# batra-mlp-lab/visdial

Measured on NVIDIA B200. Metric: QA-rounds/sec mn-att-ques-im-hist+disc train step, higher is better.
Workload: dtype f16 operands + f16 saved state for the option LSTM, tf32 operands elsewhere; fp32 accumulate, fp32 cell state / gradients / optimiser

## Files before the change

### visdial_b200/csrc/enc_lstm.cu

```cuda
#include <cuda.h>
#include <cuda_fp16.h>
#include "../../include/visdial_b200.h"
#include "kernels.cuh"
#include "tc_ptx.cuh"

namespace vd {
namespace tc {

constexpr int EP_THREADS = 192;
constexpr int EP_STAGES = 6;
constexpr int EP_STAGE_BYTES = 128 * 64 * 2;
constexpr int EP_W_BYTES_MAX = 131072;
constexpr int EP_SMEM = EP_W_BYTES_MAX + EP_STAGES * EP_STAGE_BYTES + 1024 + 256;
constexpr int EP_HS = 32;
static_assert(EP_SMEM <= 227 * 1024, "persistent encoder LSTM: shared memory budget");

__host__ __device__ constexpr uint32_t ep_idesc_f16(int M, int N) {
  return (1u << 4) | ((uint32_t)(N >> 3) << 17) | ((uint32_t)(M >> 4) << 24);
}
__device__ __forceinline__ void ep_umma_f16(uint32_t tmem_d, uint64_t adesc, uint64_t bdesc, uint32_t idesc, uint32_t accum) {
  asm volatile(
      "{\n .reg .pred p;\n setp.ne.b32 p, %4, 0;\n tcgen05.mma.cta_group::1.kind::f16 [%0], %1, %2, %3, p;\n}"
      ::"r"(tmem_d), "l"(adesc), "l"(bdesc), "r"(idesc), "r"(accum) : "memory");
}
// ... 34 lines not shown
__device__ __forceinline__ void st32h(__half* p, const float* v) {
  asm volatile("st.global.v8.b32 [%0], {%1,%2,%3,%4,%5,%6,%7,%8};"
               ::"l"(p), "r"(ep_pack2(v[0], v[1])), "r"(ep_pack2(v[2], v[3])), "r"(ep_pack2(v[4], v[5])), "r"(ep_pack2(v[6], v[7])),
                 "r"(ep_pack2(v[8], v[9])), "r"(ep_pack2(v[10], v[11])), "r"(ep_pack2(v[12], v[13])), "r"(ep_pack2(v[14], v[15])) : "memory");
  asm volatile("st.global.v8.b32 [%0], {%1,%2,%3,%4,%5,%6,%7,%8};"
               ::"l"(p + 16), "r"(ep_pack2(v[16], v[17])), "r"(ep_pack2(v[18], v[19])), "r"(ep_pack2(v[20], v[21])), "r"(ep_pack2(v[22], v[23])),
                 "r"(ep_pack2(v[24], v[25])), "r"(ep_pack2(v[26], v[27])), "r"(ep_pack2(v[28], v[29])), "r"(ep_pack2(v[30], v[31])) : "memory");
}
__device__ __forceinline__ void zero32(float* d) {
#pragma unroll
  for (int e = 0; e < 32; ++e) d[e] = 0.f;
}
__device__ __forceinline__ void tmem_ld32(uint32_t taddr, float* v) {
  tmem_ld8(taddr, v); tmem_ld8(taddr + 8, v + 8); tmem_ld8(taddr + 16, v + 16); tmem_ld8(taddr + 24, v + 24);
}
__device__ __forceinline__ void tmem_st8(uint32_t taddr, const float* v) {
  asm volatile("tcgen05.st.sync.aligned.32x32b.x8.b32 [%0], {%1,%2,%3,%4,%5,%6,%7,%8};"
               ::"r"(taddr), "r"(__float_as_uint(v[0])), "r"(__float_as_uint(v[1])), "r"(__float_as_uint(v[2])), "r"(__float_as_uint(v[3])),
                 "r"(__float_as_uint(v[4])), "r"(__float_as_uint(v[5])), "r"(__float_as_uint(v[6])), "r"(__float_as_uint(v[7])) : "memory");
}
__device__ __forceinline__ void tmem_st32(uint32_t taddr, const float* v) {
  tmem_st8(taddr, v); tmem_st8(taddr + 8, v + 8); tmem_st8(taddr + 16, v + 16); tmem_st8(taddr + 24, v + 24);
}
__device__ __forceinline__ void tmem_st_wait() { asm volatile("tcgen05.wait::st.sync.aligned;" ::: "memory"); }

constexpr int EP_TRACE_SLOTS = 10;
__device__ __forceinline__ void ep_stamp(unsigned long long* trace, int T, int t, int slot, bool wall = false) {
  if (trace) {
    unsigned long long v;
    if (wall) asm volatile("mov.u64 %0, %%globaltimer;" : "=l"(v));
    else v = (unsigned long long)clock64();
    trace[((size_t)blockIdx.x * T + t) * EP_TRACE_SLOTS + slot] = v;
  }
}

enum { EP_CELL1 = 0, EP_PROJ = 1, EP_CELL2 = 2 };

struct EncFwdParams {
  int T, R, H, RB;
// ... 645 lines not shown
```

### visdial_b200/csrc/engine.cu

```cuda
#include "engine.h"
#include <string.h>
#include <math.h>

namespace vd {

Cfg parse_cfg(const vd_params* p) {
  VD_REQUIRE(p && p->encoder && p->decoder, VD_E_BADARG, "params / encoder / decoder is null");
  Cfg c;
  c.encoder = p->encoder; c.decoder = p->decoder;
  struct { const char* name; int enc; } known[] = {
      {"lf-ques", ENC_LF_QUES}, {"lf-ques-im-hist", ENC_LF_QIH}, {"hrea-ques-im-hist", ENC_HREA}, {"mn-att-ques-im-hist", ENC_MN_ATT},
      {"lf-ques-im", ENC_LF_QI}, {"lf-ques-hist", ENC_LF_QH}, {"hre-ques-hist", ENC_HRE_QH}, {"hre-ques-im-hist", ENC_HRE_QIH},
      {"mn-ques-hist", ENC_MN_QH}, {"mn-ques-im-hist", ENC_MN_QIH}, {"lf-att-ques-im-hist", ENC_LF_ATT}};
  c.enc = -1;
  for (auto& k : known)
    if (c.encoder == k.name) c.enc = k.enc;
  VD_REQUIRE(c.enc >= 0, VD_E_BADARG, "unknown encoder (one of the eleven names of encoders/*.lua)");
  if (c.decoder == "disc") c.dec = DEC_DISC;
  else if (c.decoder == "gen") c.dec = DEC_GEN;
  else VD_REQUIRE(false, VD_E_BADARG, "unknown decoder (disc | gen)");
  c.V = p->vocabSize; c.E = p->embedSize; c.H = p->rnnHiddenSize; c.L = p->numLayers; c.F = p->imgFeatureSize;
  c.S = p->imgSpatialSize; c.IE = p->imgEmbedSize; c.Cm = p->commonEmbeddingSize; c.hops = p->numAttentionLayers;
  c.R = p->maxQuesCount; c.K = p->numOptions; c.dropout = p->dropout; c.gpuid = p->gpuid;
  c.useHist = c.encoder.find("hist") != std::string::npos;
// ... 123 lines not shown
  VD_CUDA_CHECK(cudaDeviceGetStreamPriorityRange(&prio_lo, &prio_hi));
  VD_CUDA_CHECK(cudaStreamCreateWithPriority(&cx.stream, cudaStreamNonBlocking, prio_hi));
  main_stream = cx.stream;
  VD_CUDA_CHECK(cudaStreamCreateWithPriority(&side_stream, cudaStreamNonBlocking, prio_hi));
  VD_CUDA_CHECK(cudaStreamCreateWithPriority(&main2_stream, cudaStreamNonBlocking, prio_hi));
  VD_CUDA_CHECK(cudaStreamCreateWithPriority(&side2_stream, cudaStreamNonBlocking, prio_hi));
  VD_CUDA_CHECK(cudaStreamCreateWithPriority(&main3_stream, cudaStreamNonBlocking, prio_hi));
  VD_CUDA_CHECK(cudaStreamCreateWithPriority(&side3_stream, cudaStreamNonBlocking, prio_hi));
  VD_CUDA_CHECK(cudaStreamCreateWithPriority(&opt_stream, cudaStreamNonBlocking, prio_lo));
  VD_CUDA_CHECK(cudaEventCreateWithFlags(&ev_fork, cudaEventDisableTiming));
  VD_CUDA_CHECK(cudaEventCreateWithFlags(&ev_join, cudaEventDisableTiming));
  VD_CUDA_CHECK(cudaEventCreateWithFlags(&ev_opt_fork, cudaEventDisableTiming));
  VD_CUDA_CHECK(cudaEventCreateWithFlags(&ev_opt_done, cudaEventDisableTiming));
  if (const char* s = getenv("VD_OPT_OVERLAP")) opt_overlap = atoi(s) != 0;
  if (const char* s = getenv("VD_OPT_RESERVE_SMS")) opt_reserve_sms = std::max(0, std::min(atoi(s), cx.sm_count - 16)) & ~1;
  size_t bytes = (size_t)nparams * sizeof(float);
  VD_CUDA_CHECK(cudaMalloc((void**)&W, bytes));
  VD_CUDA_CHECK(cudaMalloc((void**)&dW, bytes));
  VD_CUDA_CHECK(cudaMalloc((void**)&m, bytes));
  VD_CUDA_CHECK(cudaMalloc((void**)&v, bytes));
  VD_CUDA_CHECK(cudaMalloc((void**)&Wt, bytes));
  VD_CUDA_CHECK(cudaMemsetAsync(W, 0, bytes, cx.stream));
  VD_CUDA_CHECK(cudaMemsetAsync(dW, 0, bytes, cx.stream));
  VD_CUDA_CHECK(cudaMemsetAsync(m, 0, bytes, cx.stream));
  VD_CUDA_CHECK(cudaMemsetAsync(v, 0, bytes, cx.stream));
  VD_CUDA_CHECK(cudaMemsetAsync(Wt, 0, bytes, cx.stream));
  VD_CUDA_CHECK(cudaMalloc((void**)&scalars_dev, 64 * sizeof(float)));
  std::vector<int64_t> tab;
  for (auto& s : lay.segs) {
    if (s.init == VD_INIT_LSTM_W || s.init == VD_INIT_LINEAR_W) {
// ... 471 lines not shown
    else gemm_tn(V1, D, G, dP, G, nullptr, Ws, G, dWp(0), cfg.E, 1.f, nullptr, 0);
    VD_REQUIRE(dx_out == nullptr, VD_E_STATE, "projected-space embedding gradient: caller must not ask for dx");
    return;
  }
  if (pair16 && r.x16 && !r.gather && D % 64 == 0) {
    LaunchCtx::Scope sc(&cx, "gemm_wgrad", 2.0 * D * G * (double)TR, 2.0 * (double)TR * (D + G));
    gemm_atb16(cx, D, G, TR, r.x16, D, r.da16, G, dWs, G, nullptr);
  } else gemm_atb(D, G, TR, A, lda, r.gather, da, G, dWs, G);
  colsum_add(cx, dWp(r.wseg + 1), da, TR, G, G);
  if (dx_out) gemm_tn((int)TR, D, G, da, G, nullptr, Ws, G, dx_out, D, 0.f, nullptr, 0);
}

void Engine::lstm_backward(LstmRun& r, const float* dh_all, const float* dh_last, const float* dc_last, float* dx_out,
                           float* dh0_out, float* dc0_out) {
  lstm_backward_begin(r, dh_all, dh_last, dc_last);
  for (int t = r.T - 1; t >= 0; --t) lstm_backward_step(r, t);
  lstm_backward_end(r, dx_out, dh0_out, dc0_out);
}

void Engine::lstm_pair_backward(LstmRun& l1, LstmRun& l2, const float* dh_last2, const float* dc_last2, const float* dh_last1,
                                const float* dc_last1, float* dx1_out, cudaStream_t sa, cudaStream_t sb, cudaStream_t sc) {
  const int H = l2.H, G = 4 * l2.H;
  const int64_t R = l2.R;
  if (math_mode == VD_MATH_F16 && enc_persist_enabled() && l1.h16 && l2.h16 && l1.saved && l2.saved && l2.D == H && l1.T == l2.T &&
      enc_pair_shape_ok(R, H, cx.sm_count)) {
    const int T = l2.T;
    const int64_t TR = (int64_t)T * R;
    cx.stream = sa;
    l1.da = arena.get<float>(TR * G); l2.da = arena.get<float>(TR * G);
    l1.da16 = arena.get<__half>(TR * G); l2.da16 = arena.get<__half>(TR * G);
    __half* Whb2 = arena.get<__half>((int64_t)H * G);
// ... 746 lines not shown
```

### visdial_b200/csrc/engine.h

```cpp
#pragma once
#include <string>
#include <vector>
#include "../../include/visdial_b200.h"
#include "kernels.cuh"

namespace vd {

enum EncKind { ENC_LF_QUES = 0, ENC_LF_QIH = 1, ENC_HREA = 2, ENC_MN_ATT = 3, ENC_LF_QI = 4, ENC_LF_QH = 5, ENC_HRE_QH = 6, ENC_HRE_QIH = 7,
               ENC_MN_QH = 8, ENC_MN_QIH = 9, ENC_LF_ATT = 10 };
enum DecKind { DEC_DISC = 0, DEC_GEN = 1 };

struct Cfg {
  std::string encoder, decoder;
  int enc = 0, dec = 0;
  int V = 0, E = 300, H = 512, L = 2, F = 4096, S = 14, IE = 300, Cm = 512, hops = 1, R = 10, K = 100;
  float dropout = 0.5f;
  int gpuid = 0;
  bool useIm = false, useHist = false, att = false;
  bool fam_lf = false, fam_hre = false, fam_mn = false;
  bool hre_att = false;
  bool san = false;
  bool img_in_q = false;
  bool img_drop = false;
  bool mn_qi = false;
// ... 139 lines not shown
  void lstm_forward(LstmRun& r, bool save);
  void lstm_forward_begin(LstmRun& r, bool save);
  void lstm_forward_step(LstmRun& r, int t);
  void lstm_backward_begin(LstmRun& r, const float* dh_all, const float* dh_last, const float* dc_last);
  void lstm_backward_step(LstmRun& r, int t);
  void lstm_backward_end(LstmRun& r, float* dx_out, float* dh0_out, float* dc0_out);
  void lstm_pair_forward(LstmRun& l1, LstmRun& l2, cudaStream_t sa, cudaStream_t sb, cudaStream_t sc);
  void lstm_pair_backward(LstmRun& l1, LstmRun& l2, const float* dh_last2, const float* dc_last2, const float* dh_last1,
                          const float* dc_last1, float* dx1_out, cudaStream_t sa, cudaStream_t sb, cudaStream_t sc);
  void lstm_forward_xproj(LstmRun& r, int t);
  cudaStream_t main2_stream = nullptr, side2_stream = nullptr, main3_stream = nullptr, side3_stream = nullptr;
  cudaStream_t opt_stream = nullptr;
  cudaEvent_t ev_opt_fork = nullptr, ev_opt_done = nullptr;
  bool opt_overlap = true, opt_fwd_pending = false, opt_bwd_pending = false;
  int opt_reserve_sms = 16;
  float* opt_demb = nullptr;
  void options_forward_async();
  void join_options_backward();
  std::vector<cudaEvent_t> ev_pool;
  cudaEvent_t pool_event(size_t i);
  void lstm_backward(LstmRun& r, const float* dh_all, const float* dh_last, const float* dc_last, float* dx_out,
                     float* dh0_out, float* dc0_out);

  void encoder_forward(const vd_batch* b);
  void encoder_backward(const float* dEnc);
  float *qi_join = nullptr, *qi_proj = nullptr;
  const float* mn_query_in = nullptr;
  void mn_block_fwd(const float* qin, const float* h3, float* out);
  void mn_block_bwd(const float* dout, const float* out, float* dqin, float* dh3);
  void san_block_fwd(const float* u0);
// ... 30 lines not shown
```

### visdial_b200/csrc/kernels.cuh

```cuda
#pragma once
#include <algorithm>
#include <cuda_fp16.h>
#include "common.cuh"

namespace vd {

void gemm_tn_simt(LaunchCtx& cx, int M, int N, int K, const float* A, int64_t lda, const int32_t* a_gather,
                  const float* B, int64_t ldb, float* C, int64_t ldc, float beta, const float* bias, int act);
void gemm_atb_simt(LaunchCtx& cx, int M, int N, int64_t K, const float* A, int64_t lda, const int32_t* a_gather,
                   const float* B, int64_t ldb, float* C, int64_t ldc);
bool gemm_tn_tc(LaunchCtx& cx, int M, int N, int K, const float* A, int64_t lda, const int32_t* a_gather,
                const float* B, int64_t ldb, float* C, int64_t ldc, float beta, const float* bias, int act);
bool gemm_atb_tc(LaunchCtx& cx, int M, int N, int64_t K, const float* A, int64_t lda, const int32_t* a_gather,
                 const float* B, int64_t ldb, float* C, int64_t ldc);

int vocab_lse_nparts(int N);
bool vocab_lse_tc(LaunchCtx& cx, int M, int N, int K, const float* A, int64_t lda, const float* B, int64_t ldb, const float* bias,
                  const int32_t* tgt, float* part_max, float* part_sum, float* tgt_logit);
bool vocab_dlogits_tc(LaunchCtx& cx, int M, int N, int K, const float* A, int64_t lda, const float* B, int64_t ldb, const float* bias,
                      const int32_t* tgt, const int32_t* row_ids, const float* lse, float* C, int64_t ldc);
void vocab_lse_finish(LaunchCtx& cx, const float* part_max, const float* part_sum, int nparts, const float* tgt_logit,
                      const int32_t* tgt, const int32_t* row_ids, float* lse, float* out, float sign, int accumulate, int64_t rows);

void transpose_ids(LaunchCtx& cx, const int32_t* src, int32_t* dst, int64_t rows, int T);
// ... 79 lines not shown
bool lstm_step_fwd_tc(LaunchCtx& cx, int64_t R, int H, const float* h_prev, const float* WtS_h, int64_t ldw, const float* bias,
                      float* gates, int has_xproj, const float* ptable, const int32_t* tok, const float* c_prev, float* c_out,
                      float* h_out, const int32_t* mask_ids);
bool lstm_step_bwd_tc(LaunchCtx& cx, int64_t R, int H, const float* da_next, const float* Wh, const float* gsave,
                      const float* c_prev, const float* c_cur, const float* dh_ext, float* dc_carry, const int32_t* mask_ids,
                      float* da);
}

namespace vd {
bool lstm16_shape_ok(int64_t R, int H);
void lstm16_step_fwd(LaunchCtx& cx, int64_t R, int H, const __half* h_prev16, const __half* Wh16, const __half* ptable16,
                     const int32_t* tok, const float* bias, const float* c_prev, const int32_t* mask_ids, __half* gates16,
                     float* c_out, __half* h16_out, float* h32_out);
void lstm16_step_bwd(LaunchCtx& cx, int64_t R, int H, const __half* da_next16, const __half* Whb16, const __half* gates16,
                     const float* c_prev, const float* c_cur, float* dc_carry, const int32_t* mask_ids, __half* da16);
void lstm16_first_step(LaunchCtx& cx, int64_t R, int H, const __half* ptable16, const int32_t* tok, const float* bias,
                       const float* c_prev, const int32_t* mask_ids, __half* gates16, float* c_out, __half* h16_out, float* h32_out);
void lstm16_bwd_last(LaunchCtx& cx, int64_t R, int H, const __half* gates16, const float* c_prev, const float* c_cur,
                     const float* dh_last, const float* scale, const int32_t* mask_ids, float* dc_carry, __half* da16);
void cvt_f32_to_f16(LaunchCtx& cx, __half* dst, int64_t ldd, const float* src, int64_t lds, int64_t rows, int cols);
void pick_grad_scale(LaunchCtx& cx, const float* x, int64_t n, uint32_t* bits, float* scale2);
void segsum_rows16(LaunchCtx& cx, const __half* X, int64_t ldx, const int32_t* perm, const int32_t* sorted_tok, int64_t n,
                   float* out, int ncols, const float* inv_scale);
void gemm_atb16(LaunchCtx& cx, int M, int N, int64_t K, const __half* A, int64_t lda, const __half* B, int64_t ldb, float* C,
                int64_t ldc, const float* inv_scale);
bool enc_pair_shape_ok(int64_t R, int H, int sm_count);
void enc_pair_forward(LaunchCtx& cx, int T, int64_t R, int H, const __half* W1h16, const __half* W2cat16, const float* bias2,
                      const int32_t* mask, float* gates1, float* c1, float* h1, __half* h1_16, float* gates2, float* c2, float* h2,
                      __half* h2_16, int* flags);
void enc_pair_backward(LaunchCtx& cx, int T, int64_t R, int H, const __half* B1cat16, const __half* Whb2_16, const int32_t* mask,
// ... 7 lines not shown
```

### visdial_b200/csrc/lstm16.cu

```cuda
#include <cuda.h>
#include <cuda_fp16.h>
#include "../../include/visdial_b200.h"
#include "kernels.cuh"
#include "tc_ptx.cuh"

namespace vd {
namespace tc {

constexpr int BM16 = 128;
constexpr int BK16 = 64;
constexpr int UK16 = 16;
template <int MODE> struct EW16T { static constexpr int N = MODE == 0 ? 16 : 8; };
constexpr int STAGE16 = 32768;

__host__ __device__ constexpr uint32_t make_idesc_f16(int M, int N, int a_mn_major, int b_mn_major) {
  return (1u << 4) | ((uint32_t)a_mn_major << 15) | ((uint32_t)b_mn_major << 16) | ((uint32_t)(N >> 3) << 17) |
         ((uint32_t)(M >> 4) << 24);
}
__device__ __forceinline__ void umma_f16(uint32_t tmem_d, uint64_t adesc, uint64_t bdesc, uint32_t idesc, uint32_t accum) {
  asm volatile(
      "{\n .reg .pred p;\n setp.ne.b32 p, %4, 0;\n tcgen05.mma.cta_group::1.kind::f16 [%0], %1, %2, %3, p;\n}"
      ::"r"(tmem_d), "l"(adesc), "l"(bdesc), "r"(idesc), "r"(accum) : "memory");
}
__device__ __forceinline__ void umma_f16_cg2(uint32_t tmem_d, uint64_t adesc, uint64_t bdesc, uint32_t idesc, uint32_t accum) {
// ... 343 lines not shown
      tc_fence_before();
      __syncwarp();
      if (lane == 0) {
        if (!leader) mbar_arrive_cluster(mapa_u32(smem_u32(&tempty[buf]), 0));
        else mbar_arrive(&tempty[buf]);
      }
    }
    }
    if (lane == 0) asm volatile("cp.async.bulk.wait_group 0;" ::: "memory");
  }
  tc_fence_before();
  cluster_sync_all();
  if (warp == 1) { tc_fence_after(); tmem_dealloc_cg2(tmem_base, 2 * BN); }
}

constexpr int A16_KB = 64;
constexpr int A16_BN = 256;
constexpr int A16_THREADS = 192;
constexpr int A16_A_BYTES = 2 * A16_KB * 128;
constexpr int A16_B_BYTES = (A16_BN / 64) * A16_KB * 128;
constexpr int A16_STAGE = A16_A_BYTES + A16_B_BYTES;
constexpr int A16_STAGES = 4;
constexpr int A16_TOTAL = A16_STAGES * A16_STAGE + 1024 + 256;
struct Atb16Params { int M, N; int64_t K, k_per_split; float* C; int64_t ldc; const float* inv_scale; };

__global__ void __launch_bounds__(A16_THREADS, 1)
k_atb16(const __grid_constant__ CUtensorMap tmA, const __grid_constant__ CUtensorMap tmB, const Atb16Params p) {
  extern __shared__ uint8_t smem_raw[];
  uint8_t* smem = (uint8_t*)(((uintptr_t)smem_raw + 1023) & ~(uintptr_t)1023);
  uint64_t* full = (uint64_t*)(smem + A16_STAGES * A16_STAGE);
// ... 255 lines not shown
    snprintf(buf, sizeof(buf), "cuTensorMapEncodeTiled (lstm16) failed (%d): base %p rows %lld cols %lld ld %lld box %dx%d", (int)r, base,
             (long long)rows, (long long)cols, (long long)ld, box_rows, box_cols);
    throw CudaError(-3, buf);
  }
  return tm;
}
static CUtensorMap tmap_h(const __half* base, int64_t rows, int64_t cols, int64_t ld, int box_rows, int box_cols,
                          CUtensorMapSwizzle swz) {
  return make_tmap16(base, CU_TENSOR_MAP_DATA_TYPE_FLOAT16, 2, rows, cols, ld, box_rows, box_cols, swz);
}
static CUtensorMap tmap_f(const float* base, int64_t rows, int64_t cols, int64_t ld, int box_rows, int box_cols,
                          CUtensorMapSwizzle swz) {
  return make_tmap16(base, CU_TENSOR_MAP_DATA_TYPE_FLOAT32, 4, rows, cols, ld, box_rows, box_cols, swz);
}

template <int MODE>
static void launch16(LaunchCtx& cx, const CUtensorMap& tA, const CUtensorMap& tB, const Lstm16Maps& em, const Lstm16Params& p,
                     int num_tiles) {
  using C = Cfg16<MODE>;
  static bool attr_set = false;
  if (!attr_set) {
    VD_CUDA_CHECK(cudaFuncSetAttribute(k_lstm16<MODE>, cudaFuncAttributeMaxDynamicSharedMemorySize, C::TOTAL));
    attr_set = true;
  }
  const int pmax = cx.sms() / 2;
  int pairs = num_tiles;
  if (num_tiles > pmax) { const int rounds = cdiv(num_tiles, pmax); pairs = cdiv(num_tiles, rounds); }
  cudaLaunchConfig_t cfg = {};
  cfg.gridDim = dim3(2 * pairs);
  cfg.blockDim = dim3(C::THREADS);
  cfg.dynamicSmemBytes = C::TOTAL;
  cfg.stream = cx.stream;
  cudaLaunchAttribute at[1];
  at[0].id = cudaLaunchAttributeClusterDimension;
  at[0].val.clusterDim.x = 2; at[0].val.clusterDim.y = 1; at[0].val.clusterDim.z = 1;
  cfg.attrs = at; cfg.numAttrs = 1;
  VD_CUDA_CHECK(cudaLaunchKernelEx(&cfg, k_lstm16<MODE>, tA, tB, em, p));
  check_launch(cx, "k_lstm16");
}
// ... 23 lines not shown
void lstm16_step_bwd(LaunchCtx& cx, int64_t R, int H, const __half* da_next16, const __half* Whb16, const __half* gates16,
                     const float* c_prev, const float* c_cur, float* dc_carry, const int32_t* mask_ids, __half* da16) {
  using namespace tc;
  VD_REQUIRE(lstm16_shape_ok(R, H), VD_E_STATE, "lstm16_step_bwd: shape");
  Lstm16Params p = {};
  p.R = (int)R; p.H = H; p.gsave = gates16; p.c_prev = c_prev; p.c_cur = c_cur; p.dc_carry = dc_carry; p.mask_ids = mask_ids;
  CUtensorMap tA = tmap_h(da_next16, R, 4 * (int64_t)H, 4 * (int64_t)H, BM16, BK16, CU_TENSOR_MAP_SWIZZLE_128B);
  CUtensorMap tB = tmap_h(Whb16, H, 4 * (int64_t)H, 4 * (int64_t)H, 128, BK16, CU_TENSOR_MAP_SWIZZLE_128B);
  Lstm16Maps em;
  em.g16 = tmap_h(da16, R, 4 * (int64_t)H, 4 * (int64_t)H, 32, 16, CU_TENSOR_MAP_SWIZZLE_32B);
  em.c = tmap_f(dc_carry, R, H, H, 32, 16, CU_TENSOR_MAP_SWIZZLE_64B);
  em.h16 = em.c;
  launch16<1>(cx, tA, tB, em, p, cdiv(R, 2 * BM16) * (H / 256));
}

void lstm16_first_step(LaunchCtx& cx, int64_t R, int H, const __half* ptable16, const int32_t* tok, const float* bias,
                       const float* c_prev, const int32_t* mask_ids, __half* gates16, float* c_out, __half* h16_out, float* h32_out) {
  const int64_t n = R * (H / 8);
  tc::k_lstm16_first<<<(unsigned)((n + 255) / 256), 256, 0, cx.stream>>>(ptable16, tok, bias, c_prev, mask_ids, gates16, c_out,
                                                                          h16_out, h32_out, R, H);
  check_launch(cx, "k_lstm16_first");
}

void lstm16_bwd_last(LaunchCtx& cx, int64_t R, int H, const __half* gates16, const float* c_prev, const float* c_cur,
                     const float* dh_last, const float* scale, const int32_t* mask_ids, float* dc_carry, __half* da16) {
  const int64_t n = R * (H / 8);
  tc::k_lstm16_bwd_last<<<(unsigned)((n + 255) / 256), 256, 0, cx.stream>>>(gates16, c_prev, c_cur, dh_last, scale, mask_ids,
                                                                             dc_carry, da16, R, H);
  check_launch(cx, "k_lstm16_bwd_last");
}
// ... 25 lines not shown
  check_launch(cx, "k_segsum16");
}

void gemm_atb16(LaunchCtx& cx, int M, int N, int64_t K, const __half* A, int64_t lda, const __half* B, int64_t ldb, float* C,
                int64_t ldc, const float* inv_scale) {
  using namespace tc;
  VD_REQUIRE(M % 64 == 0 && N % 64 == 0 && K >= A16_KB && lda % 8 == 0 && ldb % 8 == 0, VD_E_STATE, "gemm_atb16: shape");
  const int tiles = cdiv(M, BM16) * cdiv(N, A16_BN);
  const int64_t cta_cap = cx.sm_budget > 0 ? cx.sm_budget : 2LL * cx.sm_count;
  int64_t splits = std::max<int64_t>(1, std::min<int64_t>(cta_cap / tiles, K / (A16_KB * 4)));
  int64_t kps = ((K + splits - 1) / splits + A16_KB - 1) / A16_KB * A16_KB;
  splits = (K + kps - 1) / kps;
  Atb16Params p = {M, N, K, kps, C, ldc, inv_scale};
  CUtensorMap tA = tmap_h(A, K, M, lda, A16_KB, 64, CU_TENSOR_MAP_SWIZZLE_128B),
              tB = tmap_h(B, K, N, ldb, A16_KB, 64, CU_TENSOR_MAP_SWIZZLE_128B);
  static bool attr_set = false;
  if (!attr_set) {
    VD_CUDA_CHECK(cudaFuncSetAttribute(k_atb16, cudaFuncAttributeMaxDynamicSharedMemorySize, A16_TOTAL));
    attr_set = true;
  }
  dim3 grid(tiles, (unsigned)splits);
  k_atb16<<<grid, A16_THREADS, A16_TOTAL, cx.stream>>>(tA, tB, p);
  check_launch(cx, "k_atb16");
}

}
```

### visdial_b200/csrc/tc_ptx.cuh

```cuda
#pragma once
#include <cuda.h>
#include <stdint.h>

namespace vd {
namespace tc {

__device__ __forceinline__ uint32_t smem_u32(const void* p) { return (uint32_t)__cvta_generic_to_shared(p); }

__device__ __forceinline__ void mbar_init(uint64_t* bar, uint32_t count) {
  asm volatile("mbarrier.init.shared::cta.b64 [%0], %1;" ::"r"(smem_u32(bar)), "r"(count));
}
__device__ __forceinline__ void mbar_expect_tx(uint64_t* bar, uint32_t bytes) {
  asm volatile("mbarrier.arrive.expect_tx.shared::cta.b64 _, [%0], %1;" ::"r"(smem_u32(bar)), "r"(bytes) : "memory");
}
__device__ __forceinline__ void mbar_arrive(uint64_t* bar) {
  asm volatile("mbarrier.arrive.shared::cta.b64 _, [%0];" ::"r"(smem_u32(bar)) : "memory");
}
__device__ __forceinline__ void mbar_wait(uint64_t* bar, uint32_t parity) {
  uint32_t done = 0, spins = 0;
  uint32_t addr = smem_u32(bar);
  while (!done) {
    asm volatile(
        "{\n .reg .pred p;\n mbarrier.try_wait.parity.shared::cta.b64 p, [%1], %2;\n selp.u32 %0, 1, 0, p;\n}"
        : "=r"(done) : "r"(addr), "r"(parity) : "memory");
// ... 51 lines not shown
  asm volatile("tcgen05.alloc.cta_group::2.sync.aligned.shared::cta.b32 [%0], %1;" ::"r"(smem_u32(dst_smem)), "r"(ncols) : "memory");
  asm volatile("tcgen05.relinquish_alloc_permit.cta_group::2.sync.aligned;" ::: "memory");
}
__device__ __forceinline__ void tmem_dealloc_cg2(uint32_t addr, uint32_t ncols) {
  asm volatile("tcgen05.dealloc.cta_group::2.sync.aligned.b32 %0, %1;" ::"r"(addr), "r"(ncols) : "memory");
}
__device__ __forceinline__ void umma_tf32_cg2(uint32_t tmem_d, uint64_t adesc, uint64_t bdesc, uint32_t idesc, uint32_t accum) {
  asm volatile(
      "{\n .reg .pred p;\n setp.ne.b32 p, %4, 0;\n tcgen05.mma.cta_group::2.kind::tf32 [%0], %1, %2, %3, p;\n}"
      ::"r"(tmem_d), "l"(adesc), "l"(bdesc), "r"(idesc), "r"(accum) : "memory");
}
__device__ __forceinline__ void umma_commit_cg2(uint64_t* bar) {
  asm volatile("tcgen05.commit.cta_group::2.mbarrier::arrive::one.shared::cluster.multicast::cluster.b64 [%0], %1;"
               ::"r"(smem_u32(bar)), "h"((uint16_t)3) : "memory");
}

__device__ __forceinline__ uint64_t make_desc(uint32_t saddr, uint32_t lbo_bytes, uint32_t sbo_bytes, uint32_t layout_type = 2) {
  uint64_t d = 0;
  d |= (uint64_t)((saddr & 0x3FFFF) >> 4);
  d |= (uint64_t)((lbo_bytes >> 4) & 0x3FFF) << 16;
  d |= (uint64_t)((sbo_bytes >> 4) & 0x3FFF) << 32;
  d |= (uint64_t)1 << 46;
  d |= (uint64_t)layout_type << 61;
  return d;
}
__host__ __device__ constexpr uint32_t make_idesc(int M, int N, int a_mn_major, int b_mn_major) {
  return (1u << 4) | (2u << 7) | (2u << 10) | ((uint32_t)a_mn_major << 15) | ((uint32_t)b_mn_major << 16) |
         ((uint32_t)(N >> 3) << 17) | ((uint32_t)(M >> 4) << 24);
}

__device__ __forceinline__ float fsigmoid(float x) { return __fdividef(1.f, 1.f + __expf(-x)); }
__device__ __forceinline__ float ftanh(float x) {
  float e = __expf(-2.f * fabsf(x));
  return copysignf(__fdividef(1.f - e, 1.f + e), x);
}

__device__ __forceinline__ const float* shfl_ptr(const float* p, int src_lane) {
  unsigned long long v = (unsigned long long)p;
  unsigned lo = __shfl_sync(0xffffffffu, (unsigned)v, src_lane), hi = __shfl_sync(0xffffffffu, (unsigned)(v >> 32), src_lane);
  return (const float*)(((unsigned long long)hi << 32) | lo);
}
__device__ __forceinline__ void tma_store_2d(const CUtensorMap* tm, const void* smem_src, int c0, int c1) {
  asm volatile("cp.async.bulk.tensor.2d.global.shared::cta.bulk_group [%0, {%2, %3}], [%1];"
               ::"l"(tm), "r"(smem_u32(smem_src)), "r"(c0), "r"(c1) : "memory");
}
__device__ __forceinline__ void fence_proxy_async_smem() { asm volatile("fence.proxy.async.shared::cta;" ::: "memory"); }
__device__ __forceinline__ void bulk_commit() { asm volatile("cp.async.bulk.commit_group;" ::: "memory"); }
__device__ __forceinline__ void bulk_wait_read0() { asm volatile("cp.async.bulk.wait_group.read 0;" ::: "memory"); }
__device__ __forceinline__ void red_add_v4(float* addr, float a, float b, float c, float d) {
  asm volatile("red.global.add.v4.f32 [%0], {%1, %2, %3, %4};" ::"l"(addr), "f"(a), "f"(b), "f"(c), "f"(d) : "memory");
}


typedef CUresult (*PFN_encodeTiled)(CUtensorMap*, CUtensorMapDataType, cuuint32_t, void*, const cuuint64_t*, const cuuint64_t*,
                                    const cuuint32_t*, const cuuint32_t*, CUtensorMapInterleave, CUtensorMapSwizzle,
                                    CUtensorMapL2promotion, CUtensorMapFloatOOBfill);
PFN_encodeTiled get_encode();
}
}
```

Baseline: 33870.

## Fuse f16 option-LSTM backward-through-time into one persistent cluster kernel

Replaces the per-timestep loop of f16 LSTM backward launches with a single persistent cluster kernel. Each step's recurrent GEMM (da_{t+1} x W_hh) runs on tcgen05 into tensor memory, and the pointwise gate gradients are computed in place, with the cell-gradient carry kept in tensor memory. Cross-CTA ordering between steps uses cluster mbarriers and TMA stores/loads. This removes T per-step launches and their global round trips for the carry, but needs the whole grid in one cluster set, adds complex cluster synchronisation, and has an environment fallback to the old path.

```diff
diff --git a/visdial_b200/csrc/enc_lstm.cu b/visdial_b200/csrc/enc_lstm.cu
--- a/visdial_b200/csrc/enc_lstm.cu
+++ b/visdial_b200/csrc/enc_lstm.cu
@@ -72,15 +72,9 @@
 __device__ __forceinline__ void tmem_ld32(uint32_t taddr, float* v) {
   tmem_ld8(taddr, v); tmem_ld8(taddr + 8, v + 8); tmem_ld8(taddr + 16, v + 16); tmem_ld8(taddr + 24, v + 24);
 }
-__device__ __forceinline__ void tmem_st8(uint32_t taddr, const float* v) {
-  asm volatile("tcgen05.st.sync.aligned.32x32b.x8.b32 [%0], {%1,%2,%3,%4,%5,%6,%7,%8};"
-               ::"r"(taddr), "r"(__float_as_uint(v[0])), "r"(__float_as_uint(v[1])), "r"(__float_as_uint(v[2])), "r"(__float_as_uint(v[3])),
-                 "r"(__float_as_uint(v[4])), "r"(__float_as_uint(v[5])), "r"(__float_as_uint(v[6])), "r"(__float_as_uint(v[7])) : "memory");
-}
 __device__ __forceinline__ void tmem_st32(uint32_t taddr, const float* v) {
   tmem_st8(taddr, v); tmem_st8(taddr + 8, v + 8); tmem_st8(taddr + 16, v + 16); tmem_st8(taddr + 24, v + 24);
 }
-__device__ __forceinline__ void tmem_st_wait() { asm volatile("tcgen05.wait::st.sync.aligned;" ::: "memory"); }
 
 constexpr int EP_TRACE_SLOTS = 10;
 __device__ __forceinline__ void ep_stamp(unsigned long long* trace, int T, int t, int slot, bool wall = false) {
diff --git a/visdial_b200/csrc/engine.cu b/visdial_b200/csrc/engine.cu
--- a/visdial_b200/csrc/engine.cu
+++ b/visdial_b200/csrc/engine.cu
@@ -161,6 +161,7 @@
   VD_CUDA_CHECK(cudaEventCreateWithFlags(&ev_opt_done, cudaEventDisableTiming));
   if (const char* s = getenv("VD_OPT_OVERLAP")) opt_overlap = atoi(s) != 0;
   if (const char* s = getenv("VD_OPT_RESERVE_SMS")) opt_reserve_sms = std::max(0, std::min(atoi(s), cx.sm_count - 16)) & ~1;
+  if (const char* s = getenv("VD_OPT_BPTT")) opt_bptt_fused = strcmp(s, "perstep") != 0;
   size_t bytes = (size_t)nparams * sizeof(float);
   VD_CUDA_CHECK(cudaMalloc((void**)&W, bytes));
   VD_CUDA_CHECK(cudaMalloc((void**)&dW, bytes));
@@ -662,7 +663,14 @@
 void Engine::lstm_backward(LstmRun& r, const float* dh_all, const float* dh_last, const float* dc_last, float* dx_out,
                            float* dh0_out, float* dc0_out) {
   lstm_backward_begin(r, dh_all, dh_last, dc_last);
-  for (int t = r.T - 1; t >= 0; --t) lstm_backward_step(r, t);
+  if (r.f16 && opt_bptt_fused && lstm16_bptt_ok(r.R, r.H, r.T)) {
+    const int H = r.H, T = r.T;
+    const double R = (double)r.R, G = 4.0 * H;
+    LaunchCtx::Scope sc(&cx, "lstm_step_bwd", (T - 1) * 2.0 * R * G * H, R * ((T - 1) * (2.0 * G + 8.0 * H + 2.0 * G) + 2.0 * G + 12.0 * H + 2.0 * G));
+    lstm16_bptt(cx, T, r.R, H, r.Whb16, r.gates16, r.c, r.c0, r.bw_dh_last, r.scale2, r.mask, r.da16);
+  } else {
+    for (int t = r.T - 1; t >= 0; --t) lstm_backward_step(r, t);
+  }
   lstm_backward_end(r, dx_out, dh0_out, dc0_out);
 }
 
diff --git a/visdial_b200/csrc/engine.h b/visdial_b200/csrc/engine.h
--- a/visdial_b200/csrc/engine.h
+++ b/visdial_b200/csrc/engine.h
@@ -177,6 +177,7 @@
   cudaEvent_t ev_opt_fork = nullptr, ev_opt_done = nullptr;
   bool opt_overlap = true, opt_fwd_pending = false, opt_bwd_pending = false;
   int opt_reserve_sms = 16;
+  bool opt_bptt_fused = true;
   float* opt_demb = nullptr;
   void options_forward_async();
   void join_options_backward();
diff --git a/visdial_b200/csrc/kernels.cuh b/visdial_b200/csrc/kernels.cuh
--- a/visdial_b200/csrc/kernels.cuh
+++ b/visdial_b200/csrc/kernels.cuh
@@ -117,6 +117,9 @@
                      float* c_out, __half* h16_out, float* h32_out);
 void lstm16_step_bwd(LaunchCtx& cx, int64_t R, int H, const __half* da_next16, const __half* Whb16, const __half* gates16,
                      const float* c_prev, const float* c_cur, float* dc_carry, const int32_t* mask_ids, __half* da16);
+bool lstm16_bptt_ok(int64_t R, int H, int T);
+void lstm16_bptt(LaunchCtx& cx,int T, int64_t R, int H, const __half* Whb16, const __half* gates16, const float* c, const float* c0,
+                 const float* dh_last, const float* scale, const int32_t* mask_ids, __half* da16);
 void lstm16_first_step(LaunchCtx& cx, int64_t R, int H, const __half* ptable16, const int32_t* tok, const float* bias,
                        const float* c_prev, const int32_t* mask_ids, __half* gates16, float* c_out, __half* h16_out, float* h32_out);
 void lstm16_bwd_last(LaunchCtx& cx, int64_t R, int H, const __half* gates16, const float* c_prev, const float* c_cur,
diff --git a/visdial_b200/csrc/lstm16.cu b/visdial_b200/csrc/lstm16.cu
--- a/visdial_b200/csrc/lstm16.cu
+++ b/visdial_b200/csrc/lstm16.cu
@@ -381,6 +381,213 @@
   if (warp == 1) { tc_fence_after(); tmem_dealloc_cg2(tmem_base, 2 * BN); }
 }
 
+struct BpttParams {
+  int R, H, T;
+  const __half* gates;
+  const float* c;
+  const float* c0;
+  const float* dh_last;
+  const float* scale;
+  const int32_t* mask;
+};
+
+__global__ void __launch_bounds__(Cfg16<1>::THREADS, 1)
+k_lstm16_bptt(const __grid_constant__ CUtensorMap tmA, const __grid_constant__ CUtensorMap tmB,
+              const __grid_constant__ CUtensorMap tmD, const BpttParams p) {
+  using C = Cfg16<1>;
+  constexpr int STAGES = C::STAGES;
+  constexpr int BN = 256;
+  const uint32_t rank = cluster_ctarank(), cs = cluster_nctarank();
+  const uint32_t lead = rank & ~1u;
+  const bool leader = rank == lead;
+  const uint16_t pair_mask = (uint16_t)(3u << lead);
+  const int sub = (int)(rank & 1), pair = (int)(rank >> 1);
+  extern __shared__ uint8_t smem_raw[];
+  uint8_t* smem = (uint8_t*)(((uintptr_t)smem_raw + 1023) & ~(uintptr_t)1023);
+  uint8_t* stg_all = smem + STAGES * STAGE16;
+  uint64_t* full = (uint64_t*)(stg_all + C::STG_BYTES);
+  uint64_t* empty = full + STAGES;
+  uint64_t* tfull = empty + STAGES;
+  uint64_t* tempty = tfull + 1;
+  uint64_t* ready = tempty + 1;
+  uint32_t* tmem_slot = (uint32_t*)(ready + 1);
+
+  const int warp = threadIdx.x >> 5, lane = threadIdx.x & 31;
+  const int H = p.H, T = p.T;
+  const int64_t R = p.R;
+  const int m0 = (int)(blockIdx.x / cs) * 2 * BM16 + sub * BM16;
+  const int n0 = pair * BN;
+  const int num_kb = 4 * H / BK16;
+
+  if (threadIdx.x == 0) {
+    for (int s = 0; s < STAGES; ++s) { mbar_init(&full[s], 1); mbar_init(&empty[s], 1); }
+    mbar_init(tfull, 1);
+    mbar_init(tempty, C::EW * 2);
+    mbar_init(ready, C::EW * cs);
+    asm volatile("fence.mbarrier_init.release.cluster;" ::: "memory");
+  }
+  cluster_sync_all();
+  if (warp == 1) tmem_alloc_cg2(tmem_slot, 2 * BN);
+  tc_fence_before();
+  __syncthreads();
+  tc_fence_after();
+  const uint32_t tmem_base = *tmem_slot;
+
+  if (warp == 0) {
+    if (lane == 0) {
+      int s = 0; uint32_t ph = 0;
+      for (int t = T - 2; t >= 0; --t) {
+        mbar_wait_acquire_cluster(ready, (uint32_t)(T - 2 - t) & 1);
+        fence_proxy_async_global();
+        for (int kb = 0; kb < num_kb; ++kb) {
+          mbar_wait(&empty[s], ph ^ 1);
+          uint8_t* sa = smem + s * STAGE16;
+          const uint32_t bar = mapa_u32(smem_u32(&full[s]), lead);
+          if (leader) mbar_expect_tx(&full[s], 2 * STAGE16);
+          tma_load_3d_cg2(sa, &tmA, bar, kb * BK16, m0, t + 1);
+          tma_load_2d_cg2(sa + 16384, &tmB, bar, kb * BK16, n0 + sub * 128);
+          if (++s == STAGES) { s = 0; ph ^= 1; }
+        }
+      }
+    }
+  } else if (warp == 1 && !leader) {
+  } else if (warp == 1) {
+    constexpr uint32_t idesc = make_idesc_f16(2 * BM16, BN, 0, 0);
+    int s = 0; uint32_t ph = 0;
+    for (int i = 0; i < T - 1; ++i) {
+      mbar_wait(tempty, ((uint32_t)i & 1) ^ 1);
+      tc_fence_after();
+      for (int kb = 0; kb < num_kb; ++kb) {
+        mbar_wait(&full[s], ph);
+        tc_fence_after();
+        if (lane == 0) {
+          const uint32_t sa = smem_u32(smem + s * STAGE16);
+          const uint64_t adesc = make_desc(sa, 16, 1024);
+          const uint64_t bdesc = make_desc(sa + 16384, 16, 1024);
+#pragma unroll
+          for (int k = 0; k < BK16 / UK16; ++k)
+            umma_f16_cg2(tmem_base, adesc + (uint64_t)(k * 2), bdesc + (uint64_t)(k * 2), idesc, (kb | k) ? 1u : 0u);
+          umma_commit_cg2_mask(&empty[s], pair_mask);
+          if (kb == num_kb - 1) umma_commit_cg2_mask(tfull, pair_mask);
+        }
+        __syncwarp();
+        if (++s == STAGES) { s = 0; ph ^= 1; }
+      }
+    }
+  } else {
+    constexpr int NSL = C::EW / 4, GPW = 256 / NSL / 16;
+    const int q = warp & 3;
+    const int half = (warp - 2) >> 2;
+    static_assert(C::EW * C::STG_PER_WARP <= STAGES * STAGE16, "second staging set must fit the pipeline stages");
+    uint8_t* const stg_a = stg_all + (warp - 2) * C::STG_PER_WARP;
+    uint8_t* const stg_b = smem + (warp - 2) * C::STG_PER_WARP;
+    const int64_t row = (int64_t)m0 + q * 32 + lane;
+    const bool row_ok = row < R;
+    const int r0 = m0 + q * 32;
+    const uint32_t taddr = tmem_base + ((uint32_t)(q * 32) << 16);
+    const float sc = __ldg(p.scale);
+    const uint32_t ready_local = smem_u32(ready);
+    for (int t = T - 1; t >= 0; --t) {
+      const bool last = t == T - 1;
+      const int64_t tr = (int64_t)t * R + row;
+      const bool masked = row_ok && p.mask && p.mask[tr] == 0;
+      const float keep = masked ? 0.f : 1.f;
+      const __half* grow = row_ok ? p.gates + tr * 4 * H : nullptr;
+      const float* cprow = !row_ok ? nullptr : t > 0 ? p.c + (tr - R) * H : p.c0 ? p.c0 + row * H : nullptr;
+      const float* ccrow = row_ok ? p.c + tr * H : nullptr;
+      const float* dhrow = (row_ok && last) ? p.dh_last + row * H : nullptr;
+      auto load_group = [&](int grp) {
+        const int j = n0 + half * (256 / NSL) + grp * 16;
+        uint8_t* b = ((grp & 1) ? stg_b : stg_a);
+        uint8_t* sCP = b + 4 * S32_BYTES; uint8_t* sCC = sCP + S64_BYTES; uint8_t* sDH = sCC + S64_BYTES;
+#pragma unroll
+        for (int g = 0; g < 4; ++g) s32_load(b + g * S32_BYTES, grow ? grow + g * H + j : nullptr, lane);
+        s64_load(sCP, cprow ? cprow + j : nullptr, lane);
+        s64_load(sCC, ccrow ? ccrow + j : nullptr, lane);
+        if (last) s64_load(sDH, dhrow ? dhrow + j : nullptr, lane);
+        asm volatile("cp.async.commit_group;" ::: "memory");
+      };
+      if (lane == 0) bulk_wait_read0();
+      __syncwarp();
+      load_group(0);
+      if (!last) { mbar_wait(tfull, (uint32_t)(T - 2 - t) & 1); tc_fence_after(); }
+#pragma unroll 1
+      for (int grp = 0; grp < GPW; ++grp) {
+        const int tc0 = half * (256 / NSL) + grp * 16;
+        const int j = n0 + tc0;
+        uint8_t* sG = ((grp & 1) ? stg_b : stg_a);
+        uint8_t* sCP = sG + 4 * S32_BYTES; uint8_t* sCC = sCP + S64_BYTES; uint8_t* sDH = sCC + S64_BYTES;
+        if (grp + 1 < GPW) {
+          if (lane == 0) bulk_wait_read0();
+          __syncwarp();
+          load_group(grp + 1);
+          asm volatile("cp.async.wait_group 1;" ::: "memory");
+        } else {
+          asm volatile("cp.async.wait_group 0;" ::: "memory");
+        }
+        __syncwarp();
+#pragma unroll 1
+        for (int sub8 = 0; sub8 < 2; ++sub8) {
+          float dh[8], g[4][8], cp[8], cc[8], dc[8], out[4][8], dcn[8];
+          if (last) {
+            s64_get8(sDH, lane, sub8, dh);
+#pragma unroll
+            for (int e = 0; e < 8; ++e) { dh[e] *= sc; dc[e] = 0.f; }
+          } else {
+            tmem_ld8(taddr + tc0 + sub8 * 8, dh);
+            tmem_ld8(taddr + BN + tc0 + sub8 * 8, dc);
+            tmem_ld_wait();
+          }
+#pragma unroll
+          for (int gg = 0; gg < 4; ++gg) unpack8(*s32_at(sG + gg * S32_BYTES, lane, sub8), g[gg]);
+          s64_get8(sCP, lane, sub8, cp);
+          s64_get8(sCC, lane, sub8, cc);
+#pragma unroll
+          for (int e = 0; e < 8; ++e) {
+            const float gi = g[0][e], gf = g[1][e], go = g[2][e], gg_ = g[3][e];
+            const float tcv = tanh16(cc[e]);
+            const float d = (dc[e] + dh[e] * go * (1.f - tcv * tcv)) * keep;
+            const float dhe = dh[e] * keep;
+            out[0][e] = d * gg_ * gi * (1.f - gi);
+            out[1][e] = d * cp[e] * gf * (1.f - gf);
+            out[2][e] = dhe * tcv * go * (1.f - go);
+            out[3][e] = d * gi * (1.f - gg_ * gg_);
+            dcn[e] = d * gf;
+          }
+#pragma unroll
+          for (int gg = 0; gg < 4; ++gg) *s32_at(sG + gg * S32_BYTES, lane, sub8) = pack8(out[gg]);
+          if (t > 0) tmem_st8(taddr + BN + tc0 + sub8 * 8, dcn);
+        }
+        if (t > 0) tmem_st_wait();
+        fence_proxy_async_smem();
+        __syncwarp();
+        if (lane == 0) {
+#pragma unroll
+          for (int gg = 0; gg < 4; ++gg) tma_store_3d(&tmD, sG + gg * S32_BYTES, gg * H + j, r0, t);
+          bulk_commit();
+        }
+        __syncwarp();
+      }
+      if (!last) {
+        tc_fence_before();
+        __syncwarp();
+        if (lane == 0) mbar_arrive_cluster(mapa_u32(smem_u32(tempty), lead));
+      }
+      if (t > 0 && lane == 0) {
+        bulk_wait0();
+        fence_proxy_async_global();
+        asm volatile("fence.acq_rel.cluster;" ::: "memory");
+        for (uint32_t r = 0; r < cs; ++r) mbar_arrive_cluster(mapa_u32(ready_local, r));
+      }
+      __syncwarp();
+    }
+    if (lane == 0) bulk_wait0();
+  }
+  tc_fence_before();
+  cluster_sync_all();
+  if (warp == 1) { tc_fence_after(); tmem_dealloc_cg2(tmem_base, 2 * BN); }
+}
+
 constexpr int A16_KB = 64;
 constexpr int A16_BN = 256;
 constexpr int A16_THREADS = 192;
@@ -666,15 +873,39 @@
   return make_tmap16(base, CU_TENSOR_MAP_DATA_TYPE_FLOAT32, 4, rows, cols, ld, box_rows, box_cols, swz);
 }
 
+static CUtensorMap tmap_h3(const __half* base, int64_t T, int64_t rows, int64_t cols, int box_rows, int box_cols,
+                           CUtensorMapSwizzle swz) {
+  CUtensorMap tm;
+  cuuint64_t dims[3] = {(cuuint64_t)cols, (cuuint64_t)rows, (cuuint64_t)T};
+  cuuint64_t strides[2] = {(cuuint64_t)cols * 2, (cuuint64_t)(rows * cols) * 2};
+  cuuint32_t box[3] = {(cuuint32_t)box_cols, (cuuint32_t)box_rows, 1};
+  cuuint32_t estr[3] = {1, 1, 1};
+  CUresult r = get_encode()(&tm, CU_TENSOR_MAP_DATA_TYPE_FLOAT16, 3, (void*)base, dims, strides, box, estr,
+                            CU_TENSOR_MAP_INTERLEAVE_NONE, swz, CU_TENSOR_MAP_L2_PROMOTION_L2_256B, CU_TENSOR_MAP_FLOAT_OOB_FILL_NONE);
+  if (r != CUDA_SUCCESS) {
+    char buf[256];
+    snprintf(buf, sizeof(buf), "cuTensorMapEncodeTiled (lstm16, 3-D) failed (%d): base %p T %lld rows %lld cols %lld box %dx%d", (int)r,
+             base, (long long)T, (long long)rows, (long long)cols, box_rows, box_cols);
+    throw CudaError(-3, buf);
+  }
+  return tm;
+}
+
+static void set_max_smem(const void* kernel, int bytes, uint64_t& done) {
+  int dev = 0;
+  VD_CUDA_CHECK(cudaGetDevice(&dev));
+  const uint64_t bit = dev < 64 ? 1ull << dev : 0;
+  if (done & bit) return;
+  VD_CUDA_CHECK(cudaFuncSetAttribute(kernel, cudaFuncAttributeMaxDynamicSharedMemorySize, bytes));
+  done |= bit;
+}
+
 template <int MODE>
 static void launch16(LaunchCtx& cx, const CUtensorMap& tA, const CUtensorMap& tB, const Lstm16Maps& em, const Lstm16Params& p,
                      int num_tiles) {
   using C = Cfg16<MODE>;
-  static bool attr_set = false;
-  if (!attr_set) {
-    VD_CUDA_CHECK(cudaFuncSetAttribute(k_lstm16<MODE>, cudaFuncAttributeMaxDynamicSharedMemorySize, C::TOTAL));
-    attr_set = true;
-  }
+  static uint64_t attr_set = 0;
+  set_max_smem((const void*)k_lstm16<MODE>, C::TOTAL, attr_set);
   const int pmax = cx.sms() / 2;
   int pairs = num_tiles;
   if (num_tiles > pmax) { const int rounds = cdiv(num_tiles, pmax); pairs = cdiv(num_tiles, rounds); }
@@ -728,6 +959,54 @@
   launch16<1>(cx, tA, tB, em, p, cdiv(R, 2 * BM16) * (H / 256));
 }
 
+static cudaLaunchConfig_t bptt_config(int64_t R, int H, cudaStream_t stream, cudaLaunchAttribute* at) {
+  using namespace tc;
+  static uint64_t attr_set = 0;
+  set_max_smem((const void*)k_lstm16_bptt, Cfg16<1>::TOTAL, attr_set);
+  const int cs = 2 * (H / 256);
+  cudaLaunchConfig_t cfg = {};
+  cfg.gridDim = dim3(cdiv(R, 2 * BM16) * cs);
+  cfg.blockDim = dim3(Cfg16<1>::THREADS);
+  cfg.dynamicSmemBytes = Cfg16<1>::TOTAL;
+  cfg.stream = stream;
+  at[0].id = cudaLaunchAttributeClusterDimension;
+  at[0].val.clusterDim.x = cs; at[0].val.clusterDim.y = 1; at[0].val.clusterDim.z = 1;
+  cfg.attrs = at; cfg.numAttrs = 1;
+  return cfg;
+}
+
+bool lstm16_bptt_ok(int64_t R, int H, int T) {
+  if (!lstm16_shape_ok(R, H) || T < 2) return false;
+  static int8_t fits[64][2] = {};
+  int dev = 0;
+  VD_CUDA_CHECK(cudaGetDevice(&dev));
+  if (dev >= 64) return false;
+  int8_t& f = fits[dev][H / 256 - 1];
+  if (f == 0) {
+    cudaLaunchAttribute at[1];
+    const cudaLaunchConfig_t cfg = bptt_config(R, H, nullptr, at);
+    int clusters = 0;
+    VD_CUDA_CHECK(cudaOccupancyMaxActiveClusters(&clusters, tc::k_lstm16_bptt, &cfg));
+    f = clusters >= 1 ? 1 : -1;
+  }
+  return f > 0;
+}
+
+void lstm16_bptt(LaunchCtx& cx, int T, int64_t R, int H, const __half* Whb16, const __half* gates16, const float* c, const float* c0,
+                 const float* dh_last, const float* scale, const int32_t* mask_ids, __half* da16) {
+  using namespace tc;
+  VD_REQUIRE(lstm16_bptt_ok(R, H, T), VD_E_STATE, "lstm16_bptt: shape");
+  BpttParams p = {(int)R, H, T, gates16, c, c0, dh_last, scale, mask_ids};
+  const int64_t G = 4 * (int64_t)H;
+  CUtensorMap tA = tmap_h3(da16, T, R, G, BM16, BK16, CU_TENSOR_MAP_SWIZZLE_128B);
+  CUtensorMap tB = tmap_h(Whb16, H, G, G, 128, BK16, CU_TENSOR_MAP_SWIZZLE_128B);
+  CUtensorMap tD = tmap_h3(da16, T, R, G, 32, 16, CU_TENSOR_MAP_SWIZZLE_32B);
+  cudaLaunchAttribute at[1];
+  const cudaLaunchConfig_t cfg = bptt_config(R, H, cx.stream, at);
+  VD_CUDA_CHECK(cudaLaunchKernelEx(&cfg, k_lstm16_bptt, tA, tB, tD, p));
+  check_launch(cx, "k_lstm16_bptt");
+}
+
 void lstm16_first_step(LaunchCtx& cx, int64_t R, int H, const __half* ptable16, const int32_t* tok, const float* bias,
                        const float* c_prev, const int32_t* mask_ids, __half* gates16, float* c_out, __half* h16_out, float* h32_out) {
   const int64_t n = R * (H / 8);
@@ -783,11 +1062,8 @@
   Atb16Params p = {M, N, K, kps, C, ldc, inv_scale};
   CUtensorMap tA = tmap_h(A, K, M, lda, A16_KB, 64, CU_TENSOR_MAP_SWIZZLE_128B),
               tB = tmap_h(B, K, N, ldb, A16_KB, 64, CU_TENSOR_MAP_SWIZZLE_128B);
-  static bool attr_set = false;
-  if (!attr_set) {
-    VD_CUDA_CHECK(cudaFuncSetAttribute(k_atb16, cudaFuncAttributeMaxDynamicSharedMemorySize, A16_TOTAL));
-    attr_set = true;
-  }
+  static uint64_t attr_set = 0;
+  set_max_smem((const void*)k_atb16, A16_TOTAL, attr_set);
   dim3 grid(tiles, (unsigned)splits);
   k_atb16<<<grid, A16_THREADS, A16_TOTAL, cx.stream>>>(tA, tB, p);
   check_launch(cx, "k_atb16");
diff --git a/visdial_b200/csrc/tc_ptx.cuh b/visdial_b200/csrc/tc_ptx.cuh
--- a/visdial_b200/csrc/tc_ptx.cuh
+++ b/visdial_b200/csrc/tc_ptx.cuh
@@ -89,6 +89,34 @@
   asm volatile("tcgen05.commit.cta_group::2.mbarrier::arrive::one.shared::cluster.multicast::cluster.b64 [%0], %1;"
                ::"r"(smem_u32(bar)), "h"((uint16_t)3) : "memory");
 }
+__device__ __forceinline__ uint32_t cluster_nctarank() { uint32_t r; asm volatile("mov.u32 %0, %%cluster_nctarank;" : "=r"(r)); return r; }
+__device__ __forceinline__ void umma_commit_cg2_mask(uint64_t* bar, uint16_t cta_mask) {
+  asm volatile("tcgen05.commit.cta_group::2.mbarrier::arrive::one.shared::cluster.multicast::cluster.b64 [%0], %1;"
+               ::"r"(smem_u32(bar)), "h"(cta_mask) : "memory");
+}
+__device__ __forceinline__ void tma_load_3d_cg2(void* smem_dst, const CUtensorMap* tm, uint32_t bar_cluster_addr, int c0, int c1, int c2) {
+  asm volatile(
+      "cp.async.bulk.tensor.3d.cta_group::2.shared::cluster.global.mbarrier::complete_tx::bytes [%0], [%1, {%3, %4, %5}], [%2];"
+      ::"r"(smem_u32(smem_dst)), "l"(tm), "r"(bar_cluster_addr), "r"(c0), "r"(c1), "r"(c2) : "memory");
+}
+__device__ __forceinline__ void tmem_st8(uint32_t taddr, const float* v) {
+  asm volatile("tcgen05.st.sync.aligned.32x32b.x8.b32 [%0], {%1,%2,%3,%4,%5,%6,%7,%8};"
+               ::"r"(taddr), "r"(__float_as_uint(v[0])), "r"(__float_as_uint(v[1])), "r"(__float_as_uint(v[2])),
+               "r"(__float_as_uint(v[3])), "r"(__float_as_uint(v[4])), "r"(__float_as_uint(v[5])), "r"(__float_as_uint(v[6])),
+               "r"(__float_as_uint(v[7])) : "memory");
+}
+__device__ __forceinline__ void tmem_st_wait() { asm volatile("tcgen05.wait::st.sync.aligned;" ::: "memory"); }
+__device__ __forceinline__ void mbar_wait_acquire_cluster(uint64_t* bar, uint32_t parity) {
+  uint32_t done = 0, spins = 0;
+  uint32_t addr = smem_u32(bar);
+  while (!done) {
+    asm volatile(
+        "{\n .reg .pred p;\n mbarrier.try_wait.parity.acquire.cluster.shared::cta.b64 p, [%1], %2;\n selp.u32 %0, 1, 0, p;\n}"
+        : "=r"(done) : "r"(addr), "r"(parity) : "memory");
+    if (!done && ++spins > (1u << 24)) __trap();
+  }
+}
+__device__ __forceinline__ void fence_proxy_async_global() { asm volatile("fence.proxy.async.global;" ::: "memory"); }
 
 __device__ __forceinline__ uint64_t make_desc(uint32_t saddr, uint32_t lbo_bytes, uint32_t sbo_bytes, uint32_t layout_type = 2) {
   uint64_t d = 0;
@@ -119,9 +147,14 @@
   asm volatile("cp.async.bulk.tensor.2d.global.shared::cta.bulk_group [%0, {%2, %3}], [%1];"
                ::"l"(tm), "r"(smem_u32(smem_src)), "r"(c0), "r"(c1) : "memory");
 }
+__device__ __forceinline__ void tma_store_3d(const CUtensorMap* tm, const void* smem_src, int c0, int c1, int c2) {
+  asm volatile("cp.async.bulk.tensor.3d.global.shared::cta.bulk_group [%0, {%2, %3, %4}], [%1];"
+               ::"l"(tm), "r"(smem_u32(smem_src)), "r"(c0), "r"(c1), "r"(c2) : "memory");
+}
 __device__ __forceinline__ void fence_proxy_async_smem() { asm volatile("fence.proxy.async.shared::cta;" ::: "memory"); }
 __device__ __forceinline__ void bulk_commit() { asm volatile("cp.async.bulk.commit_group;" ::: "memory"); }
 __device__ __forceinline__ void bulk_wait_read0() { asm volatile("cp.async.bulk.wait_group.read 0;" ::: "memory"); }
+__device__ __forceinline__ void bulk_wait0() { asm volatile("cp.async.bulk.wait_group 0;" ::: "memory"); }
 __device__ __forceinline__ void red_add_v4(float* addr, float a, float b, float c, float d) {
   asm volatile("red.global.add.v4.f32 [%0], {%1, %2, %3, %4};" ::"l"(addr), "f"(a), "f"(b), "f"(c), "f"(d) : "memory");
 }
```

After: 34650, median of 6. 2.3% higher.
